# martinsbruveris/tensorflow-image-models

Measured on NVIDIA H100. Metric: images/sec fwd bs=256 224px, higher is better.
Workload: dtype bf16

## Files before the change

tensorflow-image-models_b200/csrc/gemm_epilogue.cuh:

```cuda
#pragma once
#include "common.cuh"

namespace tfimm {

struct GemmParams {
  int M, N, K;
  const float* bias;
  const float* gamma;
  int act;
  int has_res;
  int act_post;
  void* c;
  const void* res;
  long ldc, ldr;
  const float* a_scale;
  int a_rows_per_img, a_imgs;
  int conv;
  int cv_cblocks;
  int cv_ks, cv_stride, cv_pad;
  int cv_pb, cv_ph, cv_pw;
  int cv_tiles_x, cv_tiles_y;
  int cv_B, cv_Ho, cv_Wo;
  int tk_imgs, m_out, glu;
  long img_c, img_r;
// ... 87 lines not shown
  const int lane = threadIdx.x & 31, wq = (threadIdx.x >> 5) & 3;
  const int r = wg_row0 + wq * 16 + (lane >> 2);
  const long off_c[2] = {epilogue_row_offset(p, m_blk, r, p.ldc), epilogue_row_offset(p, m_blk, r + 8, p.ldc)};
  const long off_r[2] = {p.has_res ? epilogue_row_offset(p, m_blk, r, p.ldr) : -1,
                         p.has_res ? epilogue_row_offset(p, m_blk, r + 8, p.ldr) : -1};
  OutT* __restrict__ C = reinterpret_cast<OutT*>(p.c);
  const OutT* R = reinterpret_cast<const OutT*>(p.res);
#pragma unroll
  for (int g0 = 0; g0 < BN / 8; g0 += kRun) {
    if (n_blk * BN + g0 * 8 >= p.N) break;
    uint64_t b[kRun], s[kRun], res[kRun][2];
#pragma unroll
    for (int j = 0; j < kRun; ++j) {
      const int n = n_blk * BN + (g0 + j) * 8 + 2 * (lane & 3);
      const bool in = n < p.N, two = n + 1 < p.N;
      b[j] = p.bias != nullptr ? ld_pair_or(p.bias, n, p.N, 0.f) : 0;
      s[j] = p.gamma != nullptr ? ld_pair_or(p.gamma, n, p.N, 1.f) : 0;
#pragma unroll
      for (int h = 0; h < 2; ++h)
        res[j][h] = p.has_res && in && off_r[h] >= 0 ? ld_out_pair(R + off_r[h] + n, two) : 0;
    }
#pragma unroll
    for (int j = 0; j < kRun; ++j) {
      const int g = g0 + j;
      const int n = n_blk * BN + g * 8 + 2 * (lane & 3);
      if (n_blk * BN + g * 8 >= p.N) break;
      const bool in = n < p.N, two = n + 1 < p.N;
      uint64_t v[2] = {pack2(acc[4 * g + 0], acc[4 * g + 1]), pack2(acc[4 * g + 2], acc[4 * g + 3])};
      if (p.bias != nullptr) {
        v[0] = add2(v[0], b[j]);
        v[1] = add2(v[1], b[j]);
      }
      if (!p.act_post) apply_act_pairs(v, p.act);
      if (p.gamma != nullptr) {
        v[0] = mul2(v[0], s[j]);
        v[1] = mul2(v[1], s[j]);
      }
      if (p.has_res) {
#pragma unroll
        for (int h = 0; h < 2; ++h)
          if (in && off_r[h] >= 0) v[h] = add2(v[h], res[j][h]);
      }
      if (p.act_post) apply_act_pairs(v, p.act);
#pragma unroll
      for (int h = 0; h < 2; ++h)
        if (in && off_c[h] >= 0) st_out_pair(C + off_c[h] + n, v[h], two);
    }
  }
}

template <typename OutT>
constexpr int staged_chunk_cols() { return 128 / (int)sizeof(OutT); }
constexpr int kStagedBoxBytes = 64 * 128;

template <typename OutT>
__device__ __forceinline__ uint32_t staged_addr(uint32_t s_wg, int row, int col) {
  constexpr int kCols = staged_chunk_cols<OutT>();
  const uint32_t byte = (uint32_t)(col % kCols) * (uint32_t)sizeof(OutT);
  return s_wg + (uint32_t)(col / kCols) * kStagedBoxBytes + (uint32_t)row * 128u +
         ((((byte >> 4) ^ (uint32_t)(row & 7)) << 4) | (byte & 15u));
}
__device__ __forceinline__ uint64_t ld_staged_pair(const float*, uint32_t a) {
  float x, y;
  asm volatile("ld.shared.v2.f32 {%0, %1}, [%2];" : "=f"(x), "=f"(y) : "r"(a) : "memory");
  return pack2(x, y);
}
__device__ __forceinline__ uint64_t ld_staged_pair(const __nv_bfloat16*, uint32_t a) {
  uint32_t u;
  asm volatile("ld.shared.b32 %0, [%1];" : "=r"(u) : "r"(a) : "memory");
  const float2 f = unpack_bf16x2(u);
  return pack2(f.x, f.y);
}
__device__ __forceinline__ void st_staged_pair(float*, uint32_t a, uint64_t v) {
  float x, y;
  unpack2(v, x, y);
  asm volatile("st.shared.v2.f32 [%0], {%1, %2};" ::"r"(a), "f"(x), "f"(y) : "memory");
}
__device__ __forceinline__ void st_staged_pair(__nv_bfloat16*, uint32_t a, uint64_t v) {
  float x, y;
  unpack2(v, x, y);
  asm volatile("st.shared.b32 [%0], %1;" ::"r"(a), "r"(pack_bf16x2(x, y)) : "memory");
}

template <typename OutT, int BN, int kFirst, int kSpan, int kAct>
__device__ __forceinline__ void staged_apply_act(const GemmParams& p, float (&acc)[BN / 2], uint32_t s_wg,
                                                 const float* s_bias, const float* s_gamma) {
  const int act = kAct >= 0 ? kAct : p.act;
  const int lane = threadIdx.x & 31, wq = (threadIdx.x >> 5) & 3;
  const int r = wq * 16 + (lane >> 2);
  OutT* const tag = nullptr;
#pragma unroll
  for (int g = kFirst / 8; g < (kFirst + kSpan) / 8; ++g) {
    const int c = g * 8 + 2 * (lane & 3);
    const uint32_t a0 = staged_addr<OutT>(s_wg, r, c - kFirst), a1 = a0 + 8 * 128;
    uint64_t v[2] = {pack2(acc[4 * g + 0], acc[4 * g + 1]), pack2(acc[4 * g + 2], acc[4 * g + 3])};
    if (p.bias != nullptr) {
      const float2 b = *reinterpret_cast<const float2*>(s_bias + c);
      v[0] = add2(v[0], pack2(b.x, b.y));
      v[1] = add2(v[1], pack2(b.x, b.y));
    }
    if (!p.act_post) apply_act_pairs(v, act);
    if (p.gamma != nullptr) {
      const float2 s = *reinterpret_cast<const float2*>(s_gamma + c);
      v[0] = mul2(v[0], pack2(s.x, s.y));
      v[1] = mul2(v[1], pack2(s.x, s.y));
    }
    if (p.has_res) {
      v[0] = add2(v[0], ld_staged_pair(tag, a0));
      v[1] = add2(v[1], ld_staged_pair(tag, a1));
    }
    if (p.act_post) apply_act_pairs(v, act);
    st_staged_pair(tag, a0, v[0]);
    st_staged_pair(tag, a1, v[1]);
  }
}

template <typename OutT, int BN, int kFirst, int kSpan>
__device__ __forceinline__ void staged_apply(const GemmParams& p, float (&acc)[BN / 2], uint32_t s_wg,
                                             const float* s_bias, const float* s_gamma) {
  switch (p.act) {
    case kActNone: staged_apply_act<OutT, BN, kFirst, kSpan, kActNone>(p, acc, s_wg, s_bias, s_gamma); break;
    case kActGelu: staged_apply_act<OutT, BN, kFirst, kSpan, kActGelu>(p, acc, s_wg, s_bias, s_gamma); break;
    case kActSwish: staged_apply_act<OutT, BN, kFirst, kSpan, kActSwish>(p, acc, s_wg, s_bias, s_gamma); break;
    default: staged_apply_act<OutT, BN, kFirst, kSpan, -1>(p, acc, s_wg, s_bias, s_gamma); break;
  }
}

__device__ __forceinline__ void warpgroup_bar_sync(int wg) {
  if (wg == 0) named_bar_sync<2>(128);
  else named_bar_sync<3>(128);
}

template <typename OutT, int kChunks>
__device__ __forceinline__ void staged_store(const GemmParams& p, const CUtensorMap* tmap_c, uint32_t s_wg, int row0,
                                             int col0) {
  constexpr int kCols = staged_chunk_cols<OutT>();
#pragma unroll
  for (int ch = 0; ch < kChunks; ++ch)
    if (col0 + ch * kCols < p.N) tma_store_2d(tmap_c, s_wg + (uint32_t)(ch * kStagedBoxBytes), col0 + ch * kCols, row0);
  tma_store_commit();
}

template <typename OutT, int BN>
__device__ __forceinline__ void epilogue_staged(const GemmParams& p, float (&acc)[BN / 2], int m_blk, int n_blk, int wg,
                                                uint32_t s_out, const float* s_bias, const float* s_gamma,
                                                uint32_t res_bar, const CUtensorMap* tmap_c) {
  constexpr int kChunks = BN / staged_chunk_cols<OutT>();
  const uint32_t s_wg = s_out + (uint32_t)(wg * kChunks * kStagedBoxBytes);
  named_bar_sync<1>(256);
  if (p.has_res) mbar_wait(res_bar, 0);
  staged_apply<OutT, BN, 0, BN>(p, acc, s_wg, s_bias, s_gamma);
  fence_proxy_async_smem();
  warpgroup_bar_sync(wg);
  const int row0 = m_blk * 128 + wg * 64;
  if ((threadIdx.x & 127) == 0 && row0 < p.M) {
    staged_store<OutT, kChunks>(p, tmap_c, s_wg, row0, n_blk * BN);
    tma_store_wait_read<0>();
  }
}

template <typename OutT, int BN>
__device__ __forceinline__ void epilogue_token(const GemmParams& p, float (&acc)[BN / 2], int img, int m_blk, int n_blk,
                                               int wg_row0) {
  const int lane = threadIdx.x & 31, wq = (threadIdx.x >> 5) & 3;
  const int m0 = m_blk * 128 + wg_row0 + wq * 16 + (lane >> 2);
  const float b0 = p.bias != nullptr && m0 < p.M ? __ldg(p.bias + m0) : 0.f;
  const float b1 = p.bias != nullptr && m0 + 8 < p.M ? __ldg(p.bias + m0 + 8) : 0.f;
  const int rows[2] = {p.glu ? (m0 >> 4) * 8 + (m0 & 7) : m0, p.glu ? -1 : m0 + 8};
  OutT* __restrict__ C = reinterpret_cast<OutT*>(p.c) + (long)img * p.img_c;
  const OutT* R = reinterpret_cast<const OutT*>(p.res) + (long)img * p.img_r;
  const OutT* U = reinterpret_cast<const OutT*>(p.mul) + (long)img * p.img_mul;
#pragma unroll
  for (int g = 0; g < BN / 8; ++g) {
    const int n = n_blk * BN + g * 8 + 2 * (lane & 3);
    if (n_blk * BN + g * 8 >= p.N) break;
    const bool in = n < p.N, two = n + 1 < p.N;
    uint64_t v[2] = {pack2(acc[4 * g + 0] + b0, acc[4 * g + 1] + b0), pack2(acc[4 * g + 2] + b1, acc[4 * g + 3] + b1)};
    if (p.glu) {
      float x0, x1, g0, g1;
      unpack2(v[0], x0, x1);
      unpack2(v[1], g0, g1);
      v[0] = pack2(x0 * apply_act<false>(g0, p.act), x1 * apply_act<false>(g1, p.act));
    } else {
      apply_act_pairs(v, p.act);
    }
    if (p.gamma != nullptr) {
      const uint64_t s = ld_pair_or(p.gamma, n, p.N, 1.f);
      v[0] = mul2(v[0], s);
      v[1] = mul2(v[1], s);
    }
#pragma unroll
    for (int h = 0; h < 2; ++h) {
      const int row = rows[h];
      if (!in || row < 0 || row >= p.m_out) continue;
// ... 37 lines not shown
```

tensorflow-image-models_b200/csrc/gemm_sm90.cu:

```cuda
#include <type_traits>

#include "gemm_epilogue.cuh"
#include "wgmma.cuh"

namespace tfimm {

namespace {

constexpr int kBlockM = 128;
constexpr int kRowBytes = 128;
constexpr int kConsumerThreads = 256;
constexpr int kProducerWarp = kConsumerThreads / 32;
constexpr int kNumGateWarps = 4;

enum ATransform : int {
  kANone = 0,
  kAGate = 1,
  kATf32 = 2,
};
enum GemmMode : int { kModeGemm = 0, kModeToken = 1, kModeGluCols = 2 };

template <int AX>
using OperandT = std::conditional_t<AX == kATf32, float, __nv_bfloat16>;
template <int AX>
// ... 319 lines not shown
          if (++stage == kStages) { stage = 0; phase ^= 1u; }
        }
      }
    }
    return;
  }

  const int wg = warp_idx >> 2;
  const bool leader = (threadIdx.x & 127) == 0;
  const uint32_t s_wg = smem_out + (uint32_t)(wg * Cfg::kBoxes * kStagedBoxBytes);
  const uint32_t res_bar = smem_bars + 8u * (2 * kStages + wg);
  int stage = 0, prev = 0, buf = 0;
  uint32_t phase = 0, res_phase = 0;
  for (int t = blockIdx.x; t < tiles; t += gridDim.x, buf ^= 1) {
    const int m_blk = t / num_n_tiles, n_blk = t % num_n_tiles;
    const int row0 = m_blk * kBlockM + wg * 64;
    auto has_res_span = [&](int h) { return p.has_res && row0 < p.M && n_blk * BN + h * kSpan < p.N; };
    auto load_res_span = [&](int h) {
      const int col0 = n_blk * BN + h * kSpan, chunks = min(Cfg::kBoxes, (p.N - col0 + kCols - 1) / kCols);
      mbar_expect_tx(res_bar, (uint32_t)(chunks * kStagedBoxBytes));
      for (int ch = 0; ch < chunks; ++ch)
        tma_load_2d(s_wg + (uint32_t)(ch * kStagedBoxBytes), &tmap_r, res_bar, col0 + ch * kCols, row0);
    };
    float* const s_bias = s_vec + buf * 2 * BN;
    float* const s_gamma = s_bias + BN;
    const int n_own = n_blk * BN + threadIdx.x;
    const float bias_own = p.bias != nullptr && n_own < p.N ? __ldg(p.bias + n_own) : 0.f;
    const float gamma_own = p.gamma != nullptr && n_own < p.N ? __ldg(p.gamma + n_own) : 1.f;
    float acc[BN / 2];
#pragma unroll
    for (int i = 0; i < BN / 2; ++i) acc[i] = 0.f;
    for (int kb = 0; kb < num_k_blocks; ++kb) {
      mbar_wait(full_bar(stage), phase);
      const uint32_t sa = smem_tiles + stage * Cfg::kStageBytes;
      const uint64_t da = gmma_desc_k_sw128(sa + (uint32_t)wg * (64 * 128));
      const uint64_t db = gmma_desc_k_sw128(sa + Cfg::kABytes);
      wgmma_fence();
#pragma unroll
      for (int k = 0; k < 4; ++k)
        wgmma_ss<BN, false>(acc, da + (uint64_t)(2 * k), db + (uint64_t)(2 * k), (uint32_t)((kb | k) != 0));
      wgmma_commit();
      if (kb == 0) {
        s_bias[threadIdx.x] = bias_own;
        s_gamma[threadIdx.x] = gamma_own;
      }
      if (kb == num_k_blocks / 2 && leader) {
        tma_store_wait_read<0>();
        if (has_res_span(0)) load_res_span(0);
      }
      wgmma_wait<1>();
      if (kb > 0 && leader) mbar_arrive(empty_bar(prev));
      prev = stage;
      if (++stage == kStages) { stage = 0; phase ^= 1u; }
    }
    wgmma_wait<0>();
    if (leader) mbar_arrive(empty_bar(prev));

    named_bar_sync<1>(256);
    auto span = [&](auto h_const) {
      constexpr int h = decltype(h_const)::value;
      if (n_blk * BN + h * kSpan >= p.N) return;
      if constexpr (h > 0) {
        if (leader) {
          tma_store_wait_read<0>();
          if (has_res_span(h)) load_res_span(h);
        }
        warpgroup_bar_sync(wg);
      }
      if (has_res_span(h)) {
        mbar_wait(res_bar, res_phase);
        res_phase ^= 1u;
      }
      staged_apply<OutT, BN, h * kSpan, kSpan>(p, acc, s_wg, s_bias, s_gamma);
      fence_proxy_async_smem();
      warpgroup_bar_sync(wg);
      if (leader && row0 < p.M) staged_store<OutT, Cfg::kBoxes>(p, &tmap_c, s_wg, row0, n_blk * BN + h * kSpan);
    };
    span(std::integral_constant<int, 0>{});
    if constexpr (kSpan < BN) span(std::integral_constant<int, 1>{});
  }
  if (leader) tma_store_wait_read<0>();
}

int check_out(const void* C, long ldc, const void* residual, long ldr, int esize) {
  TFIMM_CHECK_ARG((reinterpret_cast<uintptr_t>(C) & 15u) == 0 && (ldc * esize) % 16 == 0,
                  "gemm: C must be 16-byte aligned with a row stride of a multiple of 16 bytes");
  TFIMM_CHECK_ARG(residual == nullptr || ((reinterpret_cast<uintptr_t>(residual) & 15u) == 0 && (ldr * esize) % 16 == 0),
                  "gemm: residual must be 16-byte aligned with a row stride of a multiple of 16 bytes");
  return kOk;
}

template <int BLOCK_N, typename OutT, int AX, int MODE, bool STAGED = false>
int launch_wgmma(const CUtensorMap& ta, const CUtensorMap& tb, const GemmParams& p, const char* what,
                 cudaStream_t stream, const CUtensorMap& tc = CUtensorMap{}, const CUtensorMap& tr = CUtensorMap{}) {
  using Cfg = GemmCfg<BLOCK_N, OutT, STAGED>;
  auto kernel = gemm_wgmma_kernel<BLOCK_N, OutT, AX, MODE, STAGED>;
  static std::atomic<unsigned long long> attr_devs{0};
  TFIMM_CUDA_OK(set_max_dynamic_smem(kernel, Cfg::kSmemBytes, attr_devs));
  const long imgs = MODE == kModeToken ? p.tk_imgs : 1;
  const long tiles = imgs * ((p.M + kBlockM - 1) / kBlockM) * ((p.N + BLOCK_N - 1) / BLOCK_N);
  kernel<<<(unsigned)tiles, gemm_threads<BLOCK_N, AX>(), Cfg::kSmemBytes, stream>>>(ta, tb, tc, tr, p);
  TFIMM_LAUNCH_OK(what);
  return kOk;
}

template <int kMaxN, typename F>
int with_block_n(int bn, const char* unsupported_fmt, F&& launch) {
  if constexpr (kMaxN >= 256) {
    if (bn == 256) return launch(std::integral_constant<int, 256>{});
  }
  if (bn == 128) return launch(std::integral_constant<int, 128>{});
  if (bn == 64) return launch(std::integral_constant<int, 64>{});
  set_last_error(unsupported_fmt, bn);
  return kInvalidArgument;
}

template <typename OutT>
int launch_persistent(const CUtensorMap& ta, const CUtensorMap& tb, const CUtensorMap& tc, const CUtensorMap& tr,
                      const GemmParams& p, cudaStream_t stream) {
  using Cfg = PersistentCfg;
  auto kernel = gemm_persistent_kernel<OutT>;
  static std::atomic<unsigned long long> attr_devs{0};
  TFIMM_CUDA_OK(set_max_dynamic_smem(kernel, Cfg::kSmemBytes, attr_devs));
  const long tiles = (long)((p.M + kBlockM - 1) / kBlockM) * ((p.N + Cfg::kBlockN - 1) / Cfg::kBlockN);
  const int grid = (int)std::min<long>(tiles, sm_count());
  kernel<<<grid, kConsumerThreads + 32, Cfg::kSmemBytes, stream>>>(ta, tb, tc, tr, p);
  TFIMM_LAUNCH_OK("gemm_persistent_kernel (bf16)");
  return kOk;
}

template <int BLOCK_N, typename OutT, int AX = kANone, int MODE = kModeGemm, bool PERSISTENT = false>
int launch_gemm(const void* A, int lda, const void* W, int ldw, const void* residual, int ldr, void* C, int ldc,
                GemmParams p, cudaStream_t stream) {
  static_assert(!PERSISTENT || (BLOCK_N == PersistentCfg::kBlockN && AX == kANone && MODE == kModeGemm),
                "the persistent instance is the plain bf16 GEMM at 256 columns");
  const int M = p.M, N = p.N, K = p.K;
  constexpr int kBlockK = block_k<AX>();
  CUtensorMap ta, tb;
  int st;
  if ((st = check_out(C, ldc, residual, ldr, (int)sizeof(OutT))) != kOk) return st;
  if ((st = make_tmap_2d(&ta, A, dtype_code<AX>(), M, K, lda, kBlockM, kBlockK, "A")) != kOk) return st;
  if ((st = make_tmap_2d(&tb, W, dtype_code<AX>(), N, K, ldw, BLOCK_N, kBlockK, "W")) != kOk) return st;
  p.c = C; p.res = residual; p.ldc = ldc; p.ldr = ldr;
  constexpr bool kStaged = AX == kANone && MODE == kModeGemm && (BLOCK_N <= 128 || PERSISTENT);
  if constexpr (kStaged) {
    if ((long)N * (long)sizeof(OutT) % 16 != 0)
      return launch_wgmma<BLOCK_N, OutT, AX, MODE>(ta, tb, p, "gemm_wgmma_kernel (bf16)", stream);
    constexpr int es = (int)sizeof(OutT), dt = es == 2 ? kBF16 : kF32;
    CUtensorMap tc, tr{};
    if ((st = make_tmap_2d(&tc, C, dt, M, N, ldc, 64, staged_chunk_cols<OutT>(), "C")) != kOk) return st;
    if (residual != nullptr &&
        (st = make_tmap_2d(&tr, residual, dt, M, N, ldr, 64, staged_chunk_cols<OutT>(), "residual")) != kOk)
      return st;
    if constexpr (PERSISTENT) return launch_persistent<OutT>(ta, tb, tc, tr, p, stream);
    else return launch_wgmma<BLOCK_N, OutT, AX, MODE, true>(ta, tb, p, "gemm_wgmma_kernel (bf16)", stream, tc, tr);
  }
  return launch_wgmma<BLOCK_N, OutT, AX, MODE>(
      ta, tb, p,
      AX == kATf32 ? "gemm_wgmma_kernel (tf32)"
                   : (MODE == kModeGluCols ? "gemm_wgmma_kernel (bf16 glu)" : "gemm_wgmma_kernel (bf16)"),
      stream);
}

template <int BLOCK_N, typename OutT>
int launch_token(const void* Wt, int ldw, const void* X, long ldx, long img_x, GemmParams p, cudaStream_t stream) {
  CUtensorMap ta, tb;
  int st;
  if ((st = check_out(p.c, p.ldc, p.res, p.ldr, (int)sizeof(OutT))) != kOk) return st;
  if ((st = make_tmap_2d(&ta, Wt, kBF16, p.M, p.K, ldw, kBlockM, 64, "token Wt")) != kOk) return st;
  {
    const uint64_t dims[3] = {(uint64_t)p.N, (uint64_t)p.K, (uint64_t)p.tk_imgs};
    const uint64_t strides[2] = {(uint64_t)ldx * 2, (uint64_t)img_x * 2};
    const uint32_t box[3] = {64u, 64u, 1u};
    if ((st = make_tmap(&tb, X, kBF16, 3, dims, strides, box, "token X")) != kOk) return st;
  }
  return launch_wgmma<BLOCK_N, OutT, kANone, kModeToken>(ta, tb, p, "gemm_wgmma_kernel (bf16 token mixing)", stream);
}

template <int BLOCK_N, typename OutT, int AX = kANone>
int launch_conv(const void* x, const void* W, int ldw, const void* residual, void* out, int B, int H, int Wd, int C,
                int Ho, int Wo, GemmParams p, cudaStream_t stream) {
  constexpr int kBlockK = block_k<AX>();
  constexpr uint64_t es = sizeof(OperandT<AX>);
  const int N = p.N, s = p.cv_stride;
  CUtensorMap ta, tb;
  int st;
  if ((st = check_out(out, N, residual, N, (int)sizeof(OutT))) != kOk) return st;
  {
    const uint64_t dims[4] = {(uint64_t)C, (uint64_t)Wd, (uint64_t)H, (uint64_t)B};
    const uint64_t strides[3] = {(uint64_t)C * es, (uint64_t)Wd * C * es, (uint64_t)H * Wd * C * es};
    const uint32_t box[4] = {(uint32_t)kBlockK, (uint32_t)(p.cv_pw * s), (uint32_t)(p.cv_ph * s), (uint32_t)p.cv_pb};
    const uint32_t estr[4] = {1u, (uint32_t)s, (uint32_t)s, 1u};
    if ((st = make_tmap(&ta, x, dtype_code<AX>(), 4, dims, strides, box, "conv input", 128, estr)) != kOk) return st;
  }
  if ((st = make_tmap_2d(&tb, W, dtype_code<AX>(), N, p.K, ldw, BLOCK_N, kBlockK, "conv weights")) != kOk) return st;
  p.c = out; p.res = residual; p.ldc = N; p.ldr = N;
  p.cv_B = B; p.cv_Ho = Ho; p.cv_Wo = Wo;
  return launch_wgmma<BLOCK_N, OutT, AX, kModeGemm>(
      ta, tb, p,
      AX == kATf32 ? "gemm_wgmma_kernel (tf32 implicit convolution)" : "gemm_wgmma_kernel (bf16 implicit convolution)",
      stream);
}

int pick_block_n(int M, int N) {
  const int sms = sm_count() > 0 ? sm_count() : 132;
  const int mt = (M + kBlockM - 1) / kBlockM;
  int best = 256;
  double best_cost = 1e30;
  for (int bn : {256, 128, 64}) {
    const int nt = (N + bn - 1) / bn;
    const long tiles = (long)mt * nt;
    const int slots = bn == 64 ? 2 * sms : sms;
    const long waves = (tiles + slots - 1) / slots;
    const double cost = (double)waves * (bn == 64 ? 2 * bn : bn) * (bn == 256 ? 1.0 : (bn == 128 ? 1.04 : 1.10));
    if (cost < best_cost) { best_cost = cost; best = bn; }
  }
  return best;
}

constexpr int kPersistent = 1;

int pick_block_n_bf16(int M, int N, int K, int out_dtype) {
  constexpr double kEpilogueK = 926.0, kPairWidth = 184.0;
  const int sms = sm_count() > 0 ? sm_count() : 132;
  const long mt = (M + kBlockM - 1) / kBlockM;
  if (N > 256 && (out_dtype == kF32 || N % 8 == 0) && mt * ((N + 255) / 256) >= sms) return kPersistent;
  const long waves128 = (mt * ((N + 127) / 128) + sms - 1) / sms;
  const long waves64 = (mt * ((N + 63) / 64) + 2 * sms - 1) / (2 * sms);
  return (double)waves64 * kPairWidth * K < (double)waves128 * 128.0 * (K + kEpilogueK) ? 64 : 128;
}

}

int gemm_bf16_skinny(const void* A, int lda, const void* W, int ldw, const float* bias, const void* residual, int ldr,
                     void* C, int ldc, int M, int N, int K, int act, cudaStream_t stream, const float* gate = nullptr,
                     int rows_per_img = 1, int imgs = 1);

int conv_setup(GemmParams& p, const float* bias, const void* residual, int B, int H, int Wd, int C, int N, int ks,
               int stride, int pad, int act, int act_post, int cblock, int& Ho, int& Wo) {
  TFIMM_CHECK_ARG(B > 0 && H > 0 && Wd > 0 && C > 0 && C % cblock == 0, "conv: C must be a multiple of %d (got %d)",
                  cblock, C);
  TFIMM_CHECK_ARG(ks >= 1 && ks <= 7 && (stride == 1 || stride == 2) && pad >= 0 && pad < ks, "conv: bad geometry");
  TFIMM_CHECK_ARG(N > 0 && N % 8 == 0, "conv: N must be a multiple of 8 (got %d)", N);
  TFIMM_CHECK_ARG(bias == nullptr || (reinterpret_cast<uintptr_t>(bias) & 15u) == 0, "conv: bias must be 16-byte aligned");
  Ho = (H + 2 * pad - ks) / stride + 1;
  Wo = (Wd + 2 * pad - ks) / stride + 1;
  TFIMM_CHECK_ARG(Ho > 0 && Wo > 0, "conv: empty output");
  p = GemmParams{};
  p.N = N; p.K = ks * ks * C;
  p.bias = bias; p.act = act; p.has_res = residual != nullptr ? 1 : 0; p.act_post = act_post;
  p.conv = 1; p.cv_cblocks = C / cblock; p.cv_ks = ks; p.cv_stride = stride; p.cv_pad = pad;
  if (Wo > 8) { p.cv_pb = 1; p.cv_ph = 8; p.cv_pw = 16; }
  else { p.cv_pb = 2; p.cv_ph = 8; p.cv_pw = 8; }
  p.cv_tiles_x = (Wo + p.cv_pw - 1) / p.cv_pw;
  p.cv_tiles_y = (Ho + p.cv_ph - 1) / p.cv_ph;
  const int tiles_b = (B + p.cv_pb - 1) / p.cv_pb;
  p.M = tiles_b * p.cv_tiles_y * p.cv_tiles_x * kBlockM;
  return kOk;
}

}

using namespace tfimm;

extern "C" {

int tfimm_b200_gemm_bf16(const void* A, int lda, const void* W, int ldw, const float* bias, const float* gamma,
                         const void* residual, int ldr, void* C, int ldc, int M, int N, int K, int act, int act_post,
                         int out_dtype, int force_block_n, void* s) {
  const cudaStream_t stream = as_stream(s);
  TFIMM_CHECK_ARG(M > 0 && N > 0 && K > 0, "gemm: M, N, K must be positive (got %d %d %d)", M, N, K);
  TFIMM_CHECK_ARG(out_dtype == kBF16 || out_dtype == kF32, "gemm: out_dtype must be bf16 or f32");
  TFIMM_CHECK_ARG(K % 8 == 0, "gemm: K must be a multiple of 8 (got %d)", K);
  TFIMM_CHECK_ARG(bias == nullptr || (reinterpret_cast<uintptr_t>(bias) & 15u) == 0, "gemm: bias must be 16-byte aligned");
  TFIMM_CHECK_ARG(gamma == nullptr || (reinterpret_cast<uintptr_t>(gamma) & 15u) == 0, "gemm: gamma must be 16-byte aligned");
  if (force_block_n == 0 && K <= 64 && out_dtype == kBF16 && gamma == nullptr && act_post == 0) {
    const int st = gemm_bf16_skinny(A, lda, W, ldw, bias, residual, ldr, C, ldc, M, N, K, act, stream);
    if (st != kUnsupported) return st;
  }
  GemmParams p{};
  p.M = M; p.N = N; p.K = K;
  p.bias = bias; p.gamma = gamma; p.act = act; p.has_res = residual != nullptr ? 1 : 0; p.act_post = act_post;
  const int bn =
      force_block_n == 2 ? 256 : (force_block_n > 0 ? force_block_n : pick_block_n_bf16(M, N, K, out_dtype));
  if (bn == kPersistent)
    return out_dtype == kBF16
               ? launch_gemm<256, __nv_bfloat16, kANone, kModeGemm, true>(A, lda, W, ldw, residual, ldr, C, ldc, p, stream)
               : launch_gemm<256, float, kANone, kModeGemm, true>(A, lda, W, ldw, residual, ldr, C, ldc, p, stream);
  return with_block_n<256>(bn, "gemm: unsupported block_n %d", [&](auto n) {
    constexpr int BN = decltype(n)::value;
    return out_dtype == kBF16 ? launch_gemm<BN, __nv_bfloat16>(A, lda, W, ldw, residual, ldr, C, ldc, p, stream)
                              : launch_gemm<BN, float>(A, lda, W, ldw, residual, ldr, C, ldc, p, stream);
  });
}

int tfimm_b200_gemm_bf16_gated(const void* A, int lda, const float* gate, int rows_per_img, int imgs, const void* W,
                               int ldw, const float* bias, const void* residual, int ldr, void* C, int ldc, int M,
                               int N, int K, int act, void* s) {
  const cudaStream_t stream = as_stream(s);
  TFIMM_CHECK_ARG(M > 0 && N > 0 && K > 0 && K % 8 == 0, "gemm_gated: need K %% 8 == 0 (got M=%d N=%d K=%d)", M, N, K);
  TFIMM_CHECK_ARG(gate != nullptr && rows_per_img > 0 && imgs > 0 && (reinterpret_cast<uintptr_t>(gate) & 15u) == 0,
                  "gemm_gated: gate [imgs][K] fp32, 16-byte aligned");
  TFIMM_CHECK_ARG(bias == nullptr || (reinterpret_cast<uintptr_t>(bias) & 15u) == 0, "gemm_gated: bias must be 16-byte aligned");
  if (K <= 64) {
    const int st = gemm_bf16_skinny(A, lda, W, ldw, bias, residual, ldr, C, ldc, M, N, K, act, stream, gate, rows_per_img,
                                    imgs);
    if (st != kUnsupported) return st;
  }
  GemmParams p{};
  p.M = M; p.N = N; p.K = K;
  p.bias = bias; p.act = act; p.has_res = residual != nullptr ? 1 : 0;
  p.a_scale = gate; p.a_rows_per_img = rows_per_img; p.a_imgs = imgs;
  return with_block_n<128>(pick_block_n(M, N) == 64 ? 64 : 128, "gemm_gated: unsupported block_n %d", [&](auto n) {
    return launch_gemm<decltype(n)::value, __nv_bfloat16, kAGate>(A, lda, W, ldw, residual, ldr, C, ldc, p, stream);
  });
}

int tfimm_b200_conv_bf16(const void* x, const void* W, int ldw, const float* bias, const void* residual, void* out,
                         int B, int H, int Wd, int C, int N, int ks, int stride, int pad, int act, int act_post,
                         int out_dtype, void* s) {
  const cudaStream_t stream = as_stream(s);
  TFIMM_CHECK_ARG(out_dtype == kBF16 || out_dtype == kF32, "conv: out_dtype must be bf16 or f32");
  GemmParams p;
  int Ho, Wo, st;
  if ((st = conv_setup(p, bias, residual, B, H, Wd, C, N, ks, stride, pad, act, act_post, 64, Ho, Wo)) != kOk)
    return st;
  return with_block_n<256>(N >= 256 ? 256 : (N >= 128 ? 128 : 64), "conv: unsupported block_n %d", [&](auto n) {
    constexpr int BN = decltype(n)::value;
    return out_dtype == kBF16 ? launch_conv<BN, __nv_bfloat16>(x, W, ldw, residual, out, B, H, Wd, C, Ho, Wo, p, stream)
                              : launch_conv<BN, float>(x, W, ldw, residual, out, B, H, Wd, C, Ho, Wo, p, stream);
  });
}

int tfimm_b200_gemm_tf32(const float* A, int lda, const float* W, int ldw, const float* bias, const float* gamma,
                         const float* residual, int ldr, float* C, int ldc, int M, int N, int K, int act, int act_post,
                         int force_block_n, void* s) {
  const cudaStream_t stream = as_stream(s);
  TFIMM_CHECK_ARG(M > 0 && N > 0 && K > 0, "gemm_tf32: M, N, K must be positive (got %d %d %d)", M, N, K);
  TFIMM_CHECK_ARG(K % 4 == 0, "gemm_tf32: K must be a multiple of 4 (got %d)", K);
  TFIMM_CHECK_ARG(bias == nullptr || (reinterpret_cast<uintptr_t>(bias) & 15u) == 0, "gemm_tf32: bias must be 16-byte aligned");
  TFIMM_CHECK_ARG(gamma == nullptr || (reinterpret_cast<uintptr_t>(gamma) & 15u) == 0,
                  "gemm_tf32: gamma must be 16-byte aligned");
  GemmParams p{};
  p.M = M; p.N = N; p.K = K;
  p.bias = bias; p.gamma = gamma; p.act = act; p.has_res = residual != nullptr ? 1 : 0; p.act_post = act_post;
  const int bn = force_block_n == 2 ? 128 : (force_block_n > 0 ? force_block_n : (pick_block_n(M, N) == 64 ? 64 : 128));
  return with_block_n<128>(bn, "gemm_tf32: unsupported block_n %d (64 or 128)", [&](auto n) {
    return launch_gemm<decltype(n)::value, float, kATf32>(A, lda, W, ldw, residual, ldr, C, ldc, p, stream);
  });
}

int tfimm_b200_conv_tf32(const float* x, const float* W, int ldw, const float* bias, const float* residual, float* out,
                         int B, int H, int Wd, int C, int N, int ks, int stride, int pad, int act, int act_post,
                         void* s) {
  const cudaStream_t stream = as_stream(s);
  GemmParams p;
  int Ho, Wo, st;
  if ((st = conv_setup(p, bias, residual, B, H, Wd, C, N, ks, stride, pad, act, act_post, 32, Ho, Wo)) != kOk)
    return st;
  return with_block_n<128>(N >= 128 ? 128 : 64, "conv: unsupported block_n %d", [&](auto n) {
    return launch_conv<decltype(n)::value, float, kATf32>(x, W, ldw, residual, out, B, H, Wd, C, Ho, Wo, p, stream);
  });
}

int tfimm_b200_token_gemm_bf16(const void* Wt, int ldw, const void* X, long ldx, long img_x, const float* bias,
                               const float* gamma, const void* residual, long ldr, long img_r, const void* mul,
                               long ld_mul, long img_mul, void* out, long ldc, long img_c, int imgs, int M, int N,
                               int K, int m_out, int act, int glu, int out_dtype, int force_block_n, void* s) {
  const cudaStream_t stream = as_stream(s);
  TFIMM_CHECK_ARG(imgs > 0 && M > 0 && N > 0 && K > 0 && m_out > 0, "token_gemm: empty shape (imgs %d M %d N %d K %d)",
                  imgs, M, N, K);
// ... 45 lines not shown
```

tensorflow-image-models_b200/csrc/wgmma.cuh:

```cuda
#pragma once
#include <stdint.h>

namespace tfimm {

#define TFIMM_F8(i) "+f"(d[i]), "+f"(d[i + 1]), "+f"(d[i + 2]), "+f"(d[i + 3]), "+f"(d[i + 4]), "+f"(d[i + 5]), \
                    "+f"(d[i + 6]), "+f"(d[i + 7])

template <int N, int TB = 0>
__device__ __forceinline__ void wgmma_ss(float (&d)[N / 2], uint64_t a_desc, uint64_t b_desc, uint32_t accumulate);
template <int N>
__device__ __forceinline__ void wgmma_rs(float (&d)[N / 2], const uint32_t (&a)[4], uint64_t b_desc, uint32_t accumulate);

template <int TB>
__device__ __forceinline__ void wgmma_ss_n64(float (&d)[32], uint64_t a_desc, uint64_t b_desc, uint32_t accumulate) {
  asm volatile("{.reg .pred p; setp.ne.b32 p, %34, 0; wgmma.mma_async.sync.aligned.m64n64k16.f32.bf16.bf16 "
               "{%0,%1,%2,%3,%4,%5,%6,%7,%8,%9,%10,%11,%12,%13,%14,%15,%16,%17,%18,%19,"
               "%20,%21,%22,%23,%24,%25,%26,%27,%28,%29,%30,%31}, %32, %33, p, 1, 1, 0, %35;}"
               : TFIMM_F8(0), TFIMM_F8(8), TFIMM_F8(16), TFIMM_F8(24)
               : "l"(a_desc), "l"(b_desc), "r"(accumulate), "n"(TB));
}
template <int TB>
__device__ __forceinline__ void wgmma_ss_n128(float (&d)[64], uint64_t a_desc, uint64_t b_desc, uint32_t accumulate) {
  asm volatile("{.reg .pred p; setp.ne.b32 p, %66, 0; wgmma.mma_async.sync.aligned.m64n128k16.f32.bf16.bf16 "
               "{%0,%1,%2,%3,%4,%5,%6,%7,%8,%9,%10,%11,%12,%13,%14,%15,%16,%17,%18,%19,"
               "%20,%21,%22,%23,%24,%25,%26,%27,%28,%29,%30,%31,%32,%33,%34,%35,%36,%37,%38,%39,"
               "%40,%41,%42,%43,%44,%45,%46,%47,%48,%49,%50,%51,%52,%53,%54,%55,%56,%57,%58,%59,"
               "%60,%61,%62,%63}, %64, %65, p, 1, 1, 0, %67;}"
               : TFIMM_F8(0), TFIMM_F8(8), TFIMM_F8(16), TFIMM_F8(24), TFIMM_F8(32), TFIMM_F8(40),
                 TFIMM_F8(48), TFIMM_F8(56)
               : "l"(a_desc), "l"(b_desc), "r"(accumulate), "n"(TB));
}
template <int TB>
__device__ __forceinline__ void wgmma_ss_n256(float (&d)[128], uint64_t a_desc, uint64_t b_desc, uint32_t accumulate) {
  asm volatile("{.reg .pred p; setp.ne.b32 p, %130, 0; wgmma.mma_async.sync.aligned.m64n256k16.f32.bf16.bf16 "
               "{%0,%1,%2,%3,%4,%5,%6,%7,%8,%9,%10,%11,%12,%13,%14,%15,%16,%17,%18,%19,"
               "%20,%21,%22,%23,%24,%25,%26,%27,%28,%29,%30,%31,%32,%33,%34,%35,%36,%37,%38,%39,"
               "%40,%41,%42,%43,%44,%45,%46,%47,%48,%49,%50,%51,%52,%53,%54,%55,%56,%57,%58,%59,"
               "%60,%61,%62,%63,%64,%65,%66,%67,%68,%69,%70,%71,%72,%73,%74,%75,%76,%77,%78,%79,"
               "%80,%81,%82,%83,%84,%85,%86,%87,%88,%89,%90,%91,%92,%93,%94,%95,%96,%97,%98,%99,"
               "%100,%101,%102,%103,%104,%105,%106,%107,%108,%109,%110,%111,%112,%113,%114,%115,%116,%117,%118,%119,"
               "%120,%121,%122,%123,%124,%125,%126,%127}, %128, %129, p, 1, 1, 0, %131;}"
               : TFIMM_F8(0), TFIMM_F8(8), TFIMM_F8(16), TFIMM_F8(24), TFIMM_F8(32), TFIMM_F8(40),
                 TFIMM_F8(48), TFIMM_F8(56), TFIMM_F8(64), TFIMM_F8(72), TFIMM_F8(80), TFIMM_F8(88),
                 TFIMM_F8(96), TFIMM_F8(104), TFIMM_F8(112), TFIMM_F8(120)
               : "l"(a_desc), "l"(b_desc), "r"(accumulate), "n"(TB));
}
template <int N, int TB>
__device__ __forceinline__ void wgmma_ss(float (&d)[N / 2], uint64_t a_desc, uint64_t b_desc, uint32_t accumulate) {
  static_assert(N == 64 || N == 128 || N == 256, "wgmma_ss: tile width 64, 128 or 256");
  if constexpr (N == 64) wgmma_ss_n64<TB>(d, a_desc, b_desc, accumulate);
  else if constexpr (N == 128) wgmma_ss_n128<TB>(d, a_desc, b_desc, accumulate);
  else wgmma_ss_n256<TB>(d, a_desc, b_desc, accumulate);
}
template <>
__device__ __forceinline__ void wgmma_rs<96>(float (&d)[48], const uint32_t (&a)[4], uint64_t b_desc, uint32_t accumulate) {
  asm volatile("{.reg .pred p; setp.ne.b32 p, %53, 0; wgmma.mma_async.sync.aligned.m64n96k16.f32.bf16.bf16 "
               "{%0,%1,%2,%3,%4,%5,%6,%7,%8,%9,%10,%11,%12,%13,%14,%15,%16,%17,%18,%19,"
               "%20,%21,%22,%23,%24,%25,%26,%27,%28,%29,%30,%31,%32,%33,%34,%35,%36,%37,%38,%39,"
               "%40,%41,%42,%43,%44,%45,%46,%47}, {%48,%49,%50,%51}, %52, p, 1, 1, 0;}"
               : TFIMM_F8(0), TFIMM_F8(8), TFIMM_F8(16), TFIMM_F8(24), TFIMM_F8(32), TFIMM_F8(40)
               : "r"(a[0]), "r"(a[1]), "r"(a[2]), "r"(a[3]), "l"(b_desc), "r"(accumulate));
}
template <>
__device__ __forceinline__ void wgmma_rs<128>(float (&d)[64], const uint32_t (&a)[4], uint64_t b_desc, uint32_t accumulate) {
  asm volatile("{.reg .pred p; setp.ne.b32 p, %69, 0; wgmma.mma_async.sync.aligned.m64n128k16.f32.bf16.bf16 "
               "{%0,%1,%2,%3,%4,%5,%6,%7,%8,%9,%10,%11,%12,%13,%14,%15,%16,%17,%18,%19,"
               "%20,%21,%22,%23,%24,%25,%26,%27,%28,%29,%30,%31,%32,%33,%34,%35,%36,%37,%38,%39,"
               "%40,%41,%42,%43,%44,%45,%46,%47,%48,%49,%50,%51,%52,%53,%54,%55,%56,%57,%58,%59,"
               "%60,%61,%62,%63}, {%64,%65,%66,%67}, %68, p, 1, 1, 0;}"
               : TFIMM_F8(0), TFIMM_F8(8), TFIMM_F8(16), TFIMM_F8(24), TFIMM_F8(32), TFIMM_F8(40),
                 TFIMM_F8(48), TFIMM_F8(56)
               : "r"(a[0]), "r"(a[1]), "r"(a[2]), "r"(a[3]), "l"(b_desc), "r"(accumulate));
}
template <>
__device__ __forceinline__ void wgmma_rs<192>(float (&d)[96], const uint32_t (&a)[4], uint64_t b_desc, uint32_t accumulate) {
  asm volatile("{.reg .pred p; setp.ne.b32 p, %101, 0; wgmma.mma_async.sync.aligned.m64n192k16.f32.bf16.bf16 "
               "{%0,%1,%2,%3,%4,%5,%6,%7,%8,%9,%10,%11,%12,%13,%14,%15,%16,%17,%18,%19,"
               "%20,%21,%22,%23,%24,%25,%26,%27,%28,%29,%30,%31,%32,%33,%34,%35,%36,%37,%38,%39,"
               "%40,%41,%42,%43,%44,%45,%46,%47,%48,%49,%50,%51,%52,%53,%54,%55,%56,%57,%58,%59,"
               "%60,%61,%62,%63,%64,%65,%66,%67,%68,%69,%70,%71,%72,%73,%74,%75,%76,%77,%78,%79,"
               "%80,%81,%82,%83,%84,%85,%86,%87,%88,%89,%90,%91,%92,%93,%94,%95}, {%96,%97,%98,%99}, %100, p, 1, 1, 0;}"
               : TFIMM_F8(0), TFIMM_F8(8), TFIMM_F8(16), TFIMM_F8(24), TFIMM_F8(32), TFIMM_F8(40),
                 TFIMM_F8(48), TFIMM_F8(56), TFIMM_F8(64), TFIMM_F8(72), TFIMM_F8(80), TFIMM_F8(88)
               : "r"(a[0]), "r"(a[1]), "r"(a[2]), "r"(a[3]), "l"(b_desc), "r"(accumulate));
}
template <>
__device__ __forceinline__ void wgmma_rs<256>(float (&d)[128], const uint32_t (&a)[4], uint64_t b_desc, uint32_t accumulate) {
  asm volatile("{.reg .pred p; setp.ne.b32 p, %133, 0; wgmma.mma_async.sync.aligned.m64n256k16.f32.bf16.bf16 "
               "{%0,%1,%2,%3,%4,%5,%6,%7,%8,%9,%10,%11,%12,%13,%14,%15,%16,%17,%18,%19,"
               "%20,%21,%22,%23,%24,%25,%26,%27,%28,%29,%30,%31,%32,%33,%34,%35,%36,%37,%38,%39,"
               "%40,%41,%42,%43,%44,%45,%46,%47,%48,%49,%50,%51,%52,%53,%54,%55,%56,%57,%58,%59,"
               "%60,%61,%62,%63,%64,%65,%66,%67,%68,%69,%70,%71,%72,%73,%74,%75,%76,%77,%78,%79,"
               "%80,%81,%82,%83,%84,%85,%86,%87,%88,%89,%90,%91,%92,%93,%94,%95,%96,%97,%98,%99,"
               "%100,%101,%102,%103,%104,%105,%106,%107,%108,%109,%110,%111,%112,%113,%114,%115,%116,%117,%118,%119,"
               "%120,%121,%122,%123,%124,%125,%126,%127}, {%128,%129,%130,%131}, %132, p, 1, 1, 0;}"
               : TFIMM_F8(0), TFIMM_F8(8), TFIMM_F8(16), TFIMM_F8(24), TFIMM_F8(32), TFIMM_F8(40),
                 TFIMM_F8(48), TFIMM_F8(56), TFIMM_F8(64), TFIMM_F8(72), TFIMM_F8(80), TFIMM_F8(88),
                 TFIMM_F8(96), TFIMM_F8(104), TFIMM_F8(112), TFIMM_F8(120)
               : "r"(a[0]), "r"(a[1]), "r"(a[2]), "r"(a[3]), "l"(b_desc), "r"(accumulate));
}

template <int N>
__device__ __forceinline__ void wgmma_ss_tf32(float (&d)[N / 2], uint64_t a_desc, uint64_t b_desc, uint32_t accumulate);

template <>
__device__ __forceinline__ void wgmma_ss_tf32<64>(float (&d)[32], uint64_t a_desc, uint64_t b_desc,
                                                  uint32_t accumulate) {
  asm volatile("{.reg .pred p; setp.ne.b32 p, %34, 0; wgmma.mma_async.sync.aligned.m64n64k8.f32.tf32.tf32 "
               "{%0,%1,%2,%3,%4,%5,%6,%7,%8,%9,%10,%11,%12,%13,%14,%15,%16,%17,%18,%19,"
               "%20,%21,%22,%23,%24,%25,%26,%27,%28,%29,%30,%31}, %32, %33, p, 1, 1;}"
               : TFIMM_F8(0), TFIMM_F8(8), TFIMM_F8(16), TFIMM_F8(24)
               : "l"(a_desc), "l"(b_desc), "r"(accumulate));
}
template <>
__device__ __forceinline__ void wgmma_ss_tf32<128>(float (&d)[64], uint64_t a_desc, uint64_t b_desc,
                                                   uint32_t accumulate) {
  asm volatile("{.reg .pred p; setp.ne.b32 p, %66, 0; wgmma.mma_async.sync.aligned.m64n128k8.f32.tf32.tf32 "
               "{%0,%1,%2,%3,%4,%5,%6,%7,%8,%9,%10,%11,%12,%13,%14,%15,%16,%17,%18,%19,"
               "%20,%21,%22,%23,%24,%25,%26,%27,%28,%29,%30,%31,%32,%33,%34,%35,%36,%37,%38,%39,"
               "%40,%41,%42,%43,%44,%45,%46,%47,%48,%49,%50,%51,%52,%53,%54,%55,%56,%57,%58,%59,"
               "%60,%61,%62,%63}, %64, %65, p, 1, 1;}"
               : TFIMM_F8(0), TFIMM_F8(8), TFIMM_F8(16), TFIMM_F8(24), TFIMM_F8(32), TFIMM_F8(40),
                 TFIMM_F8(48), TFIMM_F8(56)
               : "l"(a_desc), "l"(b_desc), "r"(accumulate));
}

#undef TFIMM_F8

}
```

Before: 11720.

## Add persistent 192-wide GEMM kernel overlapping epilogue with next tile's MMA

```diff
diff --git a/tensorflow-image-models_b200/csrc/gemm_epilogue.cuh b/tensorflow-image-models_b200/csrc/gemm_epilogue.cuh
--- a/tensorflow-image-models_b200/csrc/gemm_epilogue.cuh
+++ b/tensorflow-image-models_b200/csrc/gemm_epilogue.cuh
@@ -193,10 +193,11 @@
   asm volatile("st.shared.b32 [%0], %1;" ::"r"(a), "r"(pack_bf16x2(x, y)) : "memory");
 }
 
-template <typename OutT, int BN, int kFirst, int kSpan, int kAct>
+template <typename OutT, int BN, int kFirst, int kSpan, int kAct, int kPost = -1>
 __device__ __forceinline__ void staged_apply_act(const GemmParams& p, float (&acc)[BN / 2], uint32_t s_wg,
                                                  const float* s_bias, const float* s_gamma) {
   const int act = kAct >= 0 ? kAct : p.act;
+  const bool post = kPost >= 0 ? kPost != 0 : p.act_post != 0;
   const int lane = threadIdx.x & 31, wq = (threadIdx.x >> 5) & 3;
   const int r = wq * 16 + (lane >> 2);
   OutT* const tag = nullptr;
@@ -210,7 +211,7 @@
       v[0] = add2(v[0], pack2(b.x, b.y));
       v[1] = add2(v[1], pack2(b.x, b.y));
     }
-    if (!p.act_post) apply_act_pairs(v, act);
+    if (!post) apply_act_pairs(v, act);
     if (p.gamma != nullptr) {
       const float2 s = *reinterpret_cast<const float2*>(s_gamma + c);
       v[0] = mul2(v[0], pack2(s.x, s.y));
@@ -220,7 +221,7 @@
       v[0] = add2(v[0], ld_staged_pair(tag, a0));
       v[1] = add2(v[1], ld_staged_pair(tag, a1));
     }
-    if (p.act_post) apply_act_pairs(v, act);
+    if (post) apply_act_pairs(v, act);
     st_staged_pair(tag, a0, v[0]);
     st_staged_pair(tag, a1, v[1]);
   }
diff --git a/tensorflow-image-models_b200/csrc/gemm_sm90.cu b/tensorflow-image-models_b200/csrc/gemm_sm90.cu
--- a/tensorflow-image-models_b200/csrc/gemm_sm90.cu
+++ b/tensorflow-image-models_b200/csrc/gemm_sm90.cu
@@ -425,6 +425,227 @@
   if (leader) tma_store_wait_read<0>();
 }
 
+struct OverlapCfg {
+  static constexpr int kBlockN = 192;
+  static constexpr int kABytes = kBlockM * kRowBytes;
+  static constexpr int kStageBytes = kABytes + kBlockN * kRowBytes;
+  static constexpr int kStages = 4;
+  static constexpr int kSlots = 3;
+  static constexpr int kAhead = 2;
+  static constexpr int kOutBytes = 2 * kSlots * kStagedBoxBytes;
+  static constexpr int kVecBytes = 2 * 2 * kBlockN * 4;
+  static constexpr int kNumBarriers = 2 * kStages + 2 * kSlots;
+  static constexpr int kSmemBytes = kStages * kStageBytes + kOutBytes + kVecBytes + kNumBarriers * 8 + 1024;
+  static constexpr int kThreads = kConsumerThreads + 128;
+  static constexpr int kProducerRegs = 40, kConsumerRegs = 232;
+};
+
+template <int N>
+__device__ __forceinline__ void setmaxnreg_dec() { asm volatile("setmaxnreg.dec.sync.aligned.u32 %0;" ::"n"(N)); }
+template <int N>
+__device__ __forceinline__ void setmaxnreg_inc() { asm volatile("setmaxnreg.inc.sync.aligned.u32 %0;" ::"n"(N)); }
+
+__device__ __forceinline__ void mbar_wait_overlap(uint32_t bar, uint32_t parity) {
+  if (mbar_try_wait(bar, parity)) return;
+  const long long t0 = clock64();
+  bool done;
+  while (!(done = mbar_try_wait(bar, parity)) && clock64() - t0 < 4000000000LL) {
+  }
+  if (!done) __trap();
+}
+
+template <int N, typename F>
+__device__ __forceinline__ void with_static_index(int i, F&& f) {
+  if constexpr (N > 0) {
+    if (i == N - 1) f(std::integral_constant<int, N - 1>{});
+    else with_static_index<N - 1>(i, f);
+  }
+}
+
+template <typename OutT, int kAct, int kPost>
+__global__ void __launch_bounds__(OverlapCfg::kThreads, 1)
+gemm_overlap_kernel(const __grid_constant__ CUtensorMap tmap_a, const __grid_constant__ CUtensorMap tmap_b,
+                    const __grid_constant__ CUtensorMap tmap_c, const __grid_constant__ CUtensorMap tmap_r,
+                    const GemmParams p) {
+  using Cfg = OverlapCfg;
+  constexpr int BN = Cfg::kBlockN, kStages = Cfg::kStages, kSlots = Cfg::kSlots, kAhead = Cfg::kAhead, kBlockK = 64;
+  constexpr int kCols = staged_chunk_cols<OutT>(), kPieces = BN / kCols;
+  static_assert(kAhead >= 1 && kAhead < kSlots && kAhead <= kPieces, "residual look-ahead");
+
+  extern __shared__ uint8_t smem_raw[];
+  const uint32_t smem_tiles = (smem_u32(smem_raw) + 1023u) & ~1023u;
+  const uint32_t smem_out = smem_tiles + kStages * Cfg::kStageBytes;
+  const uint32_t smem_vec = smem_out + Cfg::kOutBytes;
+  const uint32_t smem_bars = smem_vec + Cfg::kVecBytes;
+  auto full_bar = [&](int s) { return smem_bars + 8u * s; };
+  auto empty_bar = [&](int s) { return smem_bars + 8u * (kStages + s); };
+
+  if (threadIdx.x == kConsumerThreads) {
+    prefetch_tmap(&tmap_a);
+    prefetch_tmap(&tmap_b);
+    prefetch_tmap(&tmap_c);
+    if (p.has_res) prefetch_tmap(&tmap_r);
+    for (int s = 0; s < kStages; ++s) {
+      mbar_init(full_bar(s), 1);
+      mbar_init(empty_bar(s), 2);
+    }
+    for (int s = 0; s < 2 * kSlots; ++s) mbar_init(smem_bars + 8u * (2 * kStages + s), 1);
+    fence_mbar_init();
+  }
+  __syncthreads();
+
+  const int num_n_tiles = (p.N + BN - 1) / BN;
+  const int tiles = ((p.M + kBlockM - 1) / kBlockM) * num_n_tiles;
+  const int num_k_blocks = (p.K + kBlockK - 1) / kBlockK;
+
+  const int wg = __shfl_sync(0xffffffffu, (int)threadIdx.x >> 7, 0);
+  if (wg == 2) {
+    setmaxnreg_dec<Cfg::kProducerRegs>();
+    if (threadIdx.x == kConsumerThreads) {
+      int stage = 0;
+      uint32_t phase = 0;
+      for (int t = blockIdx.x; t < tiles; t += gridDim.x) {
+        const int m_blk = t / num_n_tiles, n_blk = t % num_n_tiles;
+        for (int kb = 0; kb < num_k_blocks; ++kb) {
+          mbar_wait_overlap(empty_bar(stage), phase ^ 1u);
+          const uint32_t sa = smem_tiles + stage * Cfg::kStageBytes;
+          mbar_expect_tx(full_bar(stage), Cfg::kStageBytes);
+          tma_load_2d(sa, &tmap_a, full_bar(stage), kb * kBlockK, m_blk * kBlockM);
+          tma_load_2d(sa + Cfg::kABytes, &tmap_b, full_bar(stage), kb * kBlockK, n_blk * BN);
+          if (++stage == kStages) { stage = 0; phase ^= 1u; }
+        }
+      }
+    }
+    return;
+  }
+  setmaxnreg_inc<Cfg::kConsumerRegs>();
+
+  const int tid = threadIdx.x & 127;
+  const bool leader = tid == 0;
+  const uint32_t s_slots = smem_out + (uint32_t)(wg * kSlots * kStagedBoxBytes);
+  const uint32_t res_bars = smem_bars + 8u * (2 * kStages + wg * kSlots);
+  float* const s_bias = reinterpret_cast<float*>(smem_raw + (smem_vec - smem_u32(smem_raw))) + wg * 2 * BN;
+  float* const s_gamma = s_bias + BN;
+  auto row0_of = [&](int t) { return (t / num_n_tiles) * kBlockM + wg * 64; };
+  auto col0_of = [&](int t) { return (t % num_n_tiles) * BN; };
+
+  auto load_box = [&](int x, int t, int b) {
+    const int s = x % kSlots;
+    const uint32_t bar = res_bars + 8u * s;
+    const int row0 = row0_of(t), col = col0_of(t) + b * kCols;
+    if (p.has_res && t < tiles && row0 < p.M && col < p.N) {
+      mbar_expect_tx(bar, kStagedBoxBytes);
+      tma_load_2d(s_slots + (uint32_t)(s * kStagedBoxBytes), &tmap_r, bar, col, row0);
+    } else {
+      mbar_arrive(bar);
+    }
+  };
+
+  int x = 0;
+  float bias_own[2] = {0.f, 0.f}, gamma_own[2] = {1.f, 1.f};
+  auto piece = [&](auto q_const, float (&acc)[BN / 2], int t) {
+    constexpr int q = decltype(q_const)::value;
+    if constexpr (q == 0) {
+      s_bias[tid] = bias_own[0];
+      s_gamma[tid] = gamma_own[0];
+      if (tid < BN - 128) {
+        s_bias[tid + 128] = bias_own[1];
+        s_gamma[tid + 128] = gamma_own[1];
+      }
+    }
+    if (leader) {
+      tma_store_wait_read<kSlots - 1 - kAhead>();
+      if constexpr (q + kAhead < kPieces) load_box(x + kAhead, t, q + kAhead);
+      else load_box(x + kAhead, t + (int)gridDim.x, q + kAhead - kPieces);
+    }
+    if constexpr (q == 0) warpgroup_bar_sync(wg);
+    const int s = x % kSlots;
+    const uint32_t slot = s_slots + (uint32_t)(s * kStagedBoxBytes);
+    const int row0 = row0_of(t), col = col0_of(t) + q * kCols;
+    mbar_wait_overlap(res_bars + 8u * s, (uint32_t)(x / kSlots) & 1u);
+    if (col < p.N) staged_apply_act<OutT, BN, q * kCols, kCols, kAct, kPost>(p, acc, slot, s_bias, s_gamma);
+    fence_proxy_async_smem();
+    warpgroup_bar_sync(wg);
+    if (leader) {
+      if (row0 < p.M && col < p.N) tma_store_2d(&tmap_c, slot, col, row0);
+      tma_store_commit();
+    }
+    ++x;
+  };
+
+  int stage = 0, pending = -1;
+  uint32_t phase = 0;
+  auto run = [&](float (&acc)[BN / 2], float (&acc_prev)[BN / 2], int t, int t_prev) __attribute__((always_inline)) {
+    auto mma_block = [&](int kb) {
+      mbar_wait_overlap(full_bar(stage), phase);
+      const uint32_t sa = smem_tiles + stage * Cfg::kStageBytes;
+      const uint64_t da = gmma_desc_k_sw128(sa + (uint32_t)wg * (64 * 128));
+      const uint64_t db = gmma_desc_k_sw128(sa + Cfg::kABytes);
+      wgmma_fence();
+#pragma unroll
+      for (int k = 0; k < 4; ++k)
+        wgmma_ss<BN, false>(acc, da + (uint64_t)(2 * k), db + (uint64_t)(2 * k), (uint32_t)((kb | k) != 0));
+      wgmma_commit();
+    };
+    auto next_stage = [&]() {
+      if (++stage == kStages) { stage = 0; phase ^= 1u; }
+    };
+    int q = kPieces;
+    if (t_prev >= 0) {
+      q = 0;
+      const int n = col0_of(t_prev) + tid;
+      bias_own[0] = p.bias != nullptr && n < p.N ? __ldg(p.bias + n) : 0.f;
+      gamma_own[0] = p.gamma != nullptr && n < p.N ? __ldg(p.gamma + n) : 1.f;
+      bias_own[1] = p.bias != nullptr && tid < BN - 128 && n + 128 < p.N ? __ldg(p.bias + n + 128) : 0.f;
+      gamma_own[1] = p.gamma != nullptr && tid < BN - 128 && n + 128 < p.N ? __ldg(p.gamma + n + 128) : 1.f;
+    }
+    const int nkb = t < tiles ? num_k_blocks : 0;
+    if (nkb > 0) mma_block(0);
+    wgmma_wait<0>();
+    if (leader && pending >= 0) mbar_arrive(empty_bar(pending));
+    pending = -1;
+    if (nkb > 0) {
+      if (leader) mbar_arrive(empty_bar(stage));
+      next_stage();
+    }
+    const int spacing = max(1, (nkb - 1) / kPieces);
+#pragma unroll 1
+    for (int kb = 1, next_kb = 1; kb < nkb || q < kPieces; ++kb) {
+      const bool mma = kb < nkb;
+      if (mma) {
+        mma_block(kb);
+        wgmma_wait<1>();
+        if (leader && pending >= 0) mbar_arrive(empty_bar(pending));
+        pending = stage;
+        next_stage();
+      }
+      if (q < kPieces && (!mma || kb == next_kb)) {
+        with_static_index<kPieces>(q, [&](auto qc) { piece(qc, acc_prev, t_prev); });
+        ++q;
+        next_kb += spacing;
+      }
+    }
+  };
+
+  float acc0[BN / 2], acc1[BN / 2];
+#pragma unroll
+  for (int i = 0; i < BN / 2; ++i) acc0[i] = acc1[i] = 0.f;
+  if (leader)
+    for (int d = 0; d < kAhead; ++d) load_box(d, blockIdx.x, d);
+  for (int t = blockIdx.x, t_prev = -1;;) {
+    run(acc0, acc1, t, t_prev);
+    if (t >= tiles) break;
+    t_prev = t;
+    t += gridDim.x;
+    run(acc1, acc0, t, t_prev);
+    if (t >= tiles) break;
+    t_prev = t;
+    t += gridDim.x;
+  }
+  wgmma_wait<0>();
+  if (leader) tma_store_wait_read<0>();
+}
+
 int check_out(const void* C, long ldc, const void* residual, long ldr, int esize) {
   TFIMM_CHECK_ARG((reinterpret_cast<uintptr_t>(C) & 15u) == 0 && (ldc * esize) % 16 == 0,
                   "gemm: C must be 16-byte aligned with a row stride of a multiple of 16 bytes");
@@ -472,11 +693,43 @@
   return kOk;
 }
 
+template <typename OutT, int kAct, int kPost>
+int launch_overlap_act(const CUtensorMap& ta, const CUtensorMap& tb, const CUtensorMap& tc, const CUtensorMap& tr,
+                       const GemmParams& p, cudaStream_t stream) {
+  using Cfg = OverlapCfg;
+  auto kernel = gemm_overlap_kernel<OutT, kAct, kPost>;
+  static std::atomic<unsigned long long> attr_devs{0};
+  TFIMM_CUDA_OK(set_max_dynamic_smem(kernel, Cfg::kSmemBytes, attr_devs));
+  const long tiles = (long)((p.M + kBlockM - 1) / kBlockM) * ((p.N + Cfg::kBlockN - 1) / Cfg::kBlockN);
+  const int grid = (int)std::min<long>(tiles, sm_count());
+  kernel<<<grid, Cfg::kThreads, Cfg::kSmemBytes, stream>>>(ta, tb, tc, tr, p);
+  TFIMM_LAUNCH_OK("gemm_overlap_kernel (bf16)");
+  return kOk;
+}
+template <typename OutT>
+int launch_overlap(const CUtensorMap& ta, const CUtensorMap& tb, const CUtensorMap& tc, const CUtensorMap& tr,
+                   const GemmParams& p, cudaStream_t stream) {
+  const bool post = p.act_post != 0;
+  switch (p.act) {
+    case kActNone: return launch_overlap_act<OutT, kActNone, -1>(ta, tb, tc, tr, p, stream);
+    case kActGelu:
+      return post ? launch_overlap_act<OutT, kActGelu, 1>(ta, tb, tc, tr, p, stream)
+                  : launch_overlap_act<OutT, kActGelu, 0>(ta, tb, tc, tr, p, stream);
+    case kActSwish:
+      return post ? launch_overlap_act<OutT, kActSwish, 1>(ta, tb, tc, tr, p, stream)
+                  : launch_overlap_act<OutT, kActSwish, 0>(ta, tb, tc, tr, p, stream);
+    default:
+      return post ? launch_overlap_act<OutT, -1, 1>(ta, tb, tc, tr, p, stream)
+                  : launch_overlap_act<OutT, -1, 0>(ta, tb, tc, tr, p, stream);
+  }
+}
+
 template <int BLOCK_N, typename OutT, int AX = kANone, int MODE = kModeGemm, bool PERSISTENT = false>
 int launch_gemm(const void* A, int lda, const void* W, int ldw, const void* residual, int ldr, void* C, int ldc,
                 GemmParams p, cudaStream_t stream) {
-  static_assert(!PERSISTENT || (BLOCK_N == PersistentCfg::kBlockN && AX == kANone && MODE == kModeGemm),
-                "the persistent instance is the plain bf16 GEMM at 256 columns");
+  static_assert(!PERSISTENT || ((BLOCK_N == PersistentCfg::kBlockN || BLOCK_N == OverlapCfg::kBlockN) && AX == kANone &&
+                                MODE == kModeGemm),
+                "the persistent instances are the plain bf16 GEMM at 256 and 192 columns");
   const int M = p.M, N = p.N, K = p.K;
   constexpr int kBlockK = block_k<AX>();
   CUtensorMap ta, tb;
@@ -495,7 +748,8 @@
     if (residual != nullptr &&
         (st = make_tmap_2d(&tr, residual, dt, M, N, ldr, 64, staged_chunk_cols<OutT>(), "residual")) != kOk)
       return st;
-    if constexpr (PERSISTENT) return launch_persistent<OutT>(ta, tb, tc, tr, p, stream);
+    if constexpr (PERSISTENT && BLOCK_N == OverlapCfg::kBlockN) return launch_overlap<OutT>(ta, tb, tc, tr, p, stream);
+    else if constexpr (PERSISTENT) return launch_persistent<OutT>(ta, tb, tc, tr, p, stream);
     else return launch_wgmma<BLOCK_N, OutT, AX, MODE, true>(ta, tb, p, "gemm_wgmma_kernel (bf16)", stream, tc, tr);
   }
   return launch_wgmma<BLOCK_N, OutT, AX, MODE>(
@@ -561,13 +815,14 @@
   return best;
 }
 
-constexpr int kPersistent = 1;
+constexpr int kPersistent = 1, kOverlap = 3;
 
 int pick_block_n_bf16(int M, int N, int K, int out_dtype) {
   constexpr double kEpilogueK = 926.0, kPairWidth = 184.0;
   const int sms = sm_count() > 0 ? sm_count() : 132;
   const long mt = (M + kBlockM - 1) / kBlockM;
-  if (N > 256 && (out_dtype == kF32 || N % 8 == 0) && mt * ((N + 255) / 256) >= sms) return kPersistent;
+  if (N > 256 && (out_dtype == kF32 || N % 8 == 0) && mt * ((N + 255) / 256) >= sms)
+    return mt * ((N + 191) / 192) >= 8L * sms ? kOverlap : kPersistent;
   const long waves128 = (mt * ((N + 127) / 128) + sms - 1) / sms;
   const long waves64 = (mt * ((N + 63) / 64) + 2 * sms - 1) / (2 * sms);
   return (double)waves64 * kPairWidth * K < (double)waves128 * 128.0 * (K + kEpilogueK) ? 64 : 128;
@@ -630,6 +885,10 @@
     return out_dtype == kBF16
                ? launch_gemm<256, __nv_bfloat16, kANone, kModeGemm, true>(A, lda, W, ldw, residual, ldr, C, ldc, p, stream)
                : launch_gemm<256, float, kANone, kModeGemm, true>(A, lda, W, ldw, residual, ldr, C, ldc, p, stream);
+  if (bn == kOverlap)
+    return out_dtype == kBF16
+               ? launch_gemm<192, __nv_bfloat16, kANone, kModeGemm, true>(A, lda, W, ldw, residual, ldr, C, ldc, p, stream)
+               : launch_gemm<192, float, kANone, kModeGemm, true>(A, lda, W, ldw, residual, ldr, C, ldc, p, stream);
   return with_block_n<256>(bn, "gemm: unsupported block_n %d", [&](auto n) {
     constexpr int BN = decltype(n)::value;
     return out_dtype == kBF16 ? launch_gemm<BN, __nv_bfloat16>(A, lda, W, ldw, residual, ldr, C, ldc, p, stream)
diff --git a/tensorflow-image-models_b200/csrc/wgmma.cuh b/tensorflow-image-models_b200/csrc/wgmma.cuh
--- a/tensorflow-image-models_b200/csrc/wgmma.cuh
+++ b/tensorflow-image-models_b200/csrc/wgmma.cuh
@@ -31,6 +31,18 @@
                : "l"(a_desc), "l"(b_desc), "r"(accumulate), "n"(TB));
 }
 template <int TB>
+__device__ __forceinline__ void wgmma_ss_n192(float (&d)[96], uint64_t a_desc, uint64_t b_desc, uint32_t accumulate) {
+  asm volatile("{.reg .pred p; setp.ne.b32 p, %98, 0; wgmma.mma_async.sync.aligned.m64n192k16.f32.bf16.bf16 "
+               "{%0,%1,%2,%3,%4,%5,%6,%7,%8,%9,%10,%11,%12,%13,%14,%15,%16,%17,%18,%19,"
+               "%20,%21,%22,%23,%24,%25,%26,%27,%28,%29,%30,%31,%32,%33,%34,%35,%36,%37,%38,%39,"
+               "%40,%41,%42,%43,%44,%45,%46,%47,%48,%49,%50,%51,%52,%53,%54,%55,%56,%57,%58,%59,"
+               "%60,%61,%62,%63,%64,%65,%66,%67,%68,%69,%70,%71,%72,%73,%74,%75,%76,%77,%78,%79,"
+               "%80,%81,%82,%83,%84,%85,%86,%87,%88,%89,%90,%91,%92,%93,%94,%95}, %96, %97, p, 1, 1, 0, %99;}"
+               : TFIMM_F8(0), TFIMM_F8(8), TFIMM_F8(16), TFIMM_F8(24), TFIMM_F8(32), TFIMM_F8(40),
+                 TFIMM_F8(48), TFIMM_F8(56), TFIMM_F8(64), TFIMM_F8(72), TFIMM_F8(80), TFIMM_F8(88)
+               : "l"(a_desc), "l"(b_desc), "r"(accumulate), "n"(TB));
+}
+template <int TB>
 __device__ __forceinline__ void wgmma_ss_n256(float (&d)[128], uint64_t a_desc, uint64_t b_desc, uint32_t accumulate) {
   asm volatile("{.reg .pred p; setp.ne.b32 p, %130, 0; wgmma.mma_async.sync.aligned.m64n256k16.f32.bf16.bf16 "
                "{%0,%1,%2,%3,%4,%5,%6,%7,%8,%9,%10,%11,%12,%13,%14,%15,%16,%17,%18,%19,"
@@ -47,9 +59,10 @@
 }
 template <int N, int TB>
 __device__ __forceinline__ void wgmma_ss(float (&d)[N / 2], uint64_t a_desc, uint64_t b_desc, uint32_t accumulate) {
-  static_assert(N == 64 || N == 128 || N == 256, "wgmma_ss: tile width 64, 128 or 256");
+  static_assert(N == 64 || N == 128 || N == 192 || N == 256, "wgmma_ss: tile width 64, 128, 192 or 256");
   if constexpr (N == 64) wgmma_ss_n64<TB>(d, a_desc, b_desc, accumulate);
   else if constexpr (N == 128) wgmma_ss_n128<TB>(d, a_desc, b_desc, accumulate);
+  else if constexpr (N == 192) wgmma_ss_n192<TB>(d, a_desc, b_desc, accumulate);
   else wgmma_ss_n256<TB>(d, a_desc, b_desc, accumulate);
 }
 template <>
```

Result: faster. 12590 (median of 6 runs) (+7.5%).
